# Gabrielcb/DaliID

Hardware: AMD Instinct MI355X
Metric: images/sec (train step) (higher is better)
Workload: dtype bf16; 1 GPU; configs[1]: ResNet-50 ReID bf16 256x128, PK batch 16x16=256 per GPU, center+proxy heads, Adam, EMA; global_batch=256, per_gpu_batch=256, parallelism=dp1

## Files before the change

daliid_amd/csrc/conv.hip:

```cpp
#include "gemm_tile.h"
#include "kernels.h"
#include <cstdlib>
#include <type_traits>
#include <vector>
#include <string>
#include <cstdio>

namespace dali {

__device__ __forceinline__ void decode_pixel(const GatherGeom& g, int p, int& n, int& ho, int& wo) {
    if (g.lhw >= 0 && g.lw >= 0) {
        n = p >> g.lhw;
        const int rem = p & ((1 << g.lhw) - 1);
        ho = rem >> g.lw;
        wo = rem & ((1 << g.lw) - 1);
    } else {
        const int hw = g.Hout * g.Wout;
        n = p / hw;
        const int rem = p - n * hw;
        ho = rem / g.Wout;
        wo = rem - ho * g.Wout;
    }
}

// ... 1049 lines not shown
        const uint16_t* sa = smem + (kt % NSTAGE) * A_ELEMS;
        const int kr = kt / 3, ks = kt - 3 * kr;
        const int tap_off = g.mode == 0 ? kr * HC + ks : (2 - kr) * HC + (2 - ks);
        uint32_t boff[FN];
#pragma unroll
        for (int j = 0; j < FN; ++j) {
            const int hp = hp_base[j] + tap_off;
            boff[j] = (uint32_t)(hp * 64 + (((lane >> 4) ^ ((hp >> 1) & 7)) << 3));
        }
#pragma unroll
        for (int h = 0; h < 2; ++h) {
            bf16x8_t fa[FM];
#pragma unroll
            for (int i = 0; i < FM; ++i) fa[i] = *reinterpret_cast<const bf16x8_t*>(sa + (i * 16) * 64 + (frag_off ^ (h << 5)));
#pragma unroll
            for (int j = 0; j < FN; ++j) {
                const bf16x8_t fb = *reinterpret_cast<const bf16x8_t*>(patch + (boff[j] ^ (uint32_t)(h << 5)));
#pragma unroll
                for (int i = 0; i < FM; ++i) acc[i][j] = __builtin_amdgcn_mfma_f32_16x16x32_bf16(fa[i], fb, acc[i][j], 0, 0, 0);
            }
        }
        asm volatile("s_waitcnt lgkmcnt(0)" ::: "memory");
        __builtin_amdgcn_s_barrier();
    }
    conv_epilogue_g<TM, TN, FM, FN, 4, NT, epi_mode(epi_fused(EPI), EPI)>(a, acc, 0, tn, smem, 0, wn);
}

}
#include "fused1x1.h"
namespace dali {

__device__ __forceinline__ int wg_swz(int row) { return (row & 3) | (((row >> 3) & 1) << 2); }

typedef short s16x4_t __attribute__((ext_vector_type(4)));

__device__ __forceinline__ int tr_frag_off(int chunk32, int lane, int half) {
    const int row = 8 * (lane >> 4) + ((lane & 15) >> 2) + 4 * half;
    return row * 128 + ((chunk32 ^ wg_swz(row)) << 4) + 4 * (lane & 3);
}
typedef short s16x8_t __attribute__((ext_vector_type(8)));
__device__ __forceinline__ bf16x8_t tr_frag(const uint16_t* tile, int chunk32, int lane) {
    typedef __attribute__((address_space(3))) s16x4_t* lds_ptr_t;
    const s16x4_t a = __builtin_amdgcn_ds_read_tr16_b64_v4i16((lds_ptr_t)(tile + tr_frag_off(chunk32, lane, 0)));
    const s16x4_t b = __builtin_amdgcn_ds_read_tr16_b64_v4i16((lds_ptr_t)(tile + tr_frag_off(chunk32, lane, 1)));
    return __builtin_bit_cast(bf16x8_t, s16x8_t{a[0], a[1], a[2], a[3], b[0], b[1], b[2], b[3]});
}

struct TrPair { s16x4_t lo, hi; };
__device__ __forceinline__ s16x4_t ds_read_tr_raw(const uint16_t* p) {
    typedef __attribute__((address_space(3))) const uint16_t* lds_cptr_t;
    const uint32_t addr = (uint32_t)(uintptr_t)(lds_cptr_t)p;
    s16x4_t v;
    asm volatile("ds_read_b64_tr_b16 %0, %1" : "=v"(v) : "v"(addr));
    return v;
}
__device__ __forceinline__ TrPair tr_frag_raw(const uint16_t* tile, int chunk32, int lane) {
    return TrPair{ds_read_tr_raw(tile + tr_frag_off(chunk32, lane, 0)), ds_read_tr_raw(tile + tr_frag_off(chunk32, lane, 1))};
}
__device__ __forceinline__ bf16x8_t tr_join(const TrPair& t) {
    return __builtin_bit_cast(bf16x8_t, s16x8_t{t.lo[0], t.lo[1], t.lo[2], t.lo[3], t.hi[0], t.hi[1], t.hi[2], t.hi[3]});
}
template <int N>
__device__ __forceinline__ void tr_settle(TrPair& a, TrPair& b, TrPair& c, TrPair& d) {
    static_assert(N == 0 || N == 8 || N == 10 || N == 16 || N == 18, "lgkmcnt immediates used by the callers");
    asm volatile("s_waitcnt lgkmcnt(%8)" : "+v"(a.lo), "+v"(a.hi), "+v"(b.lo), "+v"(b.hi), "+v"(c.lo), "+v"(c.hi), "+v"(d.lo), "+v"(d.hi) : "n"(N > 15 ? 15 : N));
}

__device__ __forceinline__ void tr_settle_all(TrPair& a) { asm volatile("s_waitcnt lgkmcnt(0)" : "+v"(a.lo), "+v"(a.hi)); }

template <int FM, int FN>
__device__ __forceinline__ void store_slab_tiles(float* slab, const f32x4_t (&acc)[FM][FN], int m_first, int n_first, int Cm, int Ntot, int lane) {
    const int mr = m_first + (lane >> 4) * 4, nc = n_first + (lane & 15);
    if (m_first + 16 * FM <= Cm && n_first + 16 * FN <= Ntot) {
        float* row = slab + (size_t)mr * Ntot + nc;
#pragma unroll
        for (int i = 0; i < FM; ++i)
#pragma unroll
            for (int rr = 0; rr < 4; ++rr) {
                float* p = row + (size_t)(i * 16 + rr) * Ntot;
#pragma unroll
                for (int j = 0; j < FN; ++j) p[j * 16] = acc[i][j][rr];
            }
        return;
    }
#pragma unroll
    for (int i = 0; i < FM; ++i)
#pragma unroll
        for (int j = 0; j < FN; ++j) {
            const int n = nc + j * 16;
#pragma unroll
            for (int rr = 0; rr < 4; ++rr) {
                const int m = mr + i * 16 + rr;
                if (m < Cm && n < Ntot) slab[(size_t)m * Ntot + n] = acc[i][j][rr];
// ... 1477 lines not shown
```

daliid_amd/csrc/gemm_tile.h:

```cpp
#pragma once
#include "common.h"

namespace dali {

__device__ __forceinline__ int lds_swz(int row) { return (0x1320 >> (((row >> 2) & 3) * 4)) & 3; }

template <int TM_, int TN_, int NA_, int NB_, int NPROD_>
struct GemmCfg {
    static constexpr int TM = TM_, TN = TN_, NA = NA_, NB = NB_, NPROD = NPROD_;
    static constexpr int BK = 32;
    static constexpr int FM = TM / 32, FN = TN / 32;
    static constexpr int A_ELEMS = TM * BK, B_ELEMS = TN * BK;
    static constexpr int STAGE_ELEMS = NA * A_ELEMS + NB * B_ELEMS;
    static constexpr int LDS_BYTES = 2 * STAGE_ELEMS * 2;
    static constexpr int ACH = TM * 4 / 256, BCH = TN * 4 / 256;
    static_assert(TM % 64 == 0 && TN % 64 == 0, "tile must be a multiple of 64");
    static_assert(NPROD == 1 || (NPROD == 3 && NA == 2 && NB == 2), "NPROD 3 needs hi/lo on both operands");
};

template <class Cfg, class LA, class LB>
__device__ __forceinline__ void gemm_mainloop(f32x4_t (&acc)[Cfg::FM][Cfg::FN], const LA& la, const LB& lb,
                                              int ktiles, uint16_t* smem) {
    constexpr int FM = Cfg::FM, FN = Cfg::FN, NA = Cfg::NA, NB = Cfg::NB;
    const int tid = threadIdx.x, lane = tid & 63, wave = tid >> 6;
// ... 64 lines not shown
                acc[i][j] = __builtin_amdgcn_mfma_f32_16x16x32_bf16(fa[0][i], fb[0], acc[i][j], 0, 0, 0);
                if constexpr (Cfg::NPROD == 3) {
                    acc[i][j] = __builtin_amdgcn_mfma_f32_16x16x32_bf16(fa[0][i], fb[1], acc[i][j], 0, 0, 0);
                    acc[i][j] = __builtin_amdgcn_mfma_f32_16x16x32_bf16(fa[1][i], fb[0], acc[i][j], 0, 0, 0);
                }
            }
        }
        if (more) sstore((kt + 1) & 1);
        __syncthreads();
    }
}

template <class Cfg>
__device__ __forceinline__ void acc_coords(int& m_base, int& n_base) {
    const int lane = threadIdx.x & 63, wave = threadIdx.x >> 6;
    m_base = (wave >> 1) * (Cfg::TM / 2) + (lane >> 4) * 4;
    n_base = (wave & 1) * (Cfg::TN / 2) + (lane & 15);
}

typedef __attribute__((address_space(3))) void* lds_void_ptr;
constexpr uint32_t DMA_OOB = 0x7ffffff0u;

template <int N>
__device__ __forceinline__ void vm_wait() {
    static_assert(N >= 0 && N <= 63, "vmcnt is a 6-bit field");
    asm volatile("s_waitcnt vmcnt(%0)" ::"n"(N) : "memory");
}
template <int N>
__device__ __forceinline__ void dma_wait() {
    static_assert(N == 0 || N == 2 || N == 3 || N == 4 || N == 5 || N == 6 || N == 8 || N == 9 || N == 10 || N == 12, "DMA piece counts of the rings in use");
    asm volatile("s_waitcnt vmcnt(%0) lgkmcnt(0)" ::"n"(N) : "memory");
}

__host__ __device__ __forceinline__ void xcd_super_shape(int tiles_m, int tiles_n, int& lg, int& ms) {
    const long long total = (long long)tiles_m * tiles_n;
    lg = total >= 1024 ? 6 : total >= 512 ? 5 : total >= 256 ? 4 : 3;
    ms = tiles_m >= 5 ? 3 : tiles_m >= 3 ? 2 : tiles_m == 2 ? 1 : 0;
    if (ms > lg) ms = lg;
}
__host__ __device__ __forceinline__ bool xcd_dense_map(int tiles_m, int ms) { return (tiles_m & ((1 << ms) - 1)) != 0; }
__device__ __forceinline__ bool xcd_tile_map(int b, int tiles_m, int tiles_n, int& tm, int& tn) {
    int lg, ms;
    xcd_super_shape(tiles_m, tiles_n, lg, ms);
    if (xcd_dense_map(tiles_m, ms)) {
        const int BM = tiles_m <= 16 ? tiles_m : 8;
        const int T = tiles_m * tiles_n, per = (T + 7) >> 3;
        const int xcd = b & 7, slot = b >> 3;
        const int t = xcd * per + slot;
        if (slot >= per || t >= T) return false;
        const int band_tiles = BM * tiles_n;
        const int band = t / band_tiles;
        const int r = t - band * band_tiles;
        const int left = tiles_m - band * BM;
        const int h = left < BM ? left : BM;
        tn = r / h;
        tm = band * BM + (r - tn * h);
        return true;
    }
    const int ns = lg - ms;
    const int xcd = b & 7, slot = b >> 3;
    const int ssn = (tiles_n + (1 << ns) - 1) >> ns;
    const int st = (slot >> lg) * 8 + xcd;
    const int w = slot & ((1 << lg) - 1);
    const int sm = st / ssn, sn = st - sm * ssn;
    tm = (sm << ms) + (w & ((1 << ms) - 1));
    tn = (sn << ns) + (w >> ms);
// ... 14 lines not shown
```

daliid_amd/csrc/kernels.h:

```cpp
#pragma once
#include "common.h"

namespace dali {

struct GatherGeom {
    int Hout, Wout;
    int Hin, Win;
    int Ck;
    int R, S, stride, pad;
    int mode;
    long long img_pitch;
    int row_pitch, pix_pitch;
    int lw, lhw;
    int sub, oph, opw, Hfull, Wfull;
    int r0, rstep, nr, s0, sstep, ns;
    int class_grid;
};

struct IGemmArgs {
    const uint16_t* W;
    const uint16_t* X;
    uint16_t* O;
    const uint16_t* Res;
    const uint8_t* res_mask;
// ... 60 lines not shown
int launch_bnlin_stats(hipStream_t st, const uint16_t* W, const uint16_t* Wt, const float* gram, const float* m2, int C, int w, double count, const float* gamma,
                       const float* beta, float* rm, float* rv, float momentum, float eps, float* ut, float* dot, float* scale, float* shift,
                       float* mean, float* invstd);
int launch_bnlin_ut(hipStream_t st, const uint16_t* W, const float* gram, int C, int w, float* ut);
int launch_bnlin_bwd(hipStream_t st, const uint16_t* W, const uint16_t* Wt, const float* ut, const float* m2, const float* s_dz, int C,
                     int w, double count, const float* scale, const float* mean, const float* invstd, float* dW, float* dgamma, float* dbeta,
                     uint16_t* wd1, uint16_t* wd2, float* bvec, float* qk, int ld1 = 0, int ld2 = 0);

constexpr int REDUCE_SMAX = 64;
inline size_t reduce_scratch_bytes(int C, int NV) { return (size_t)REDUCE_SMAX * C * NV * sizeof(double); }
int launch_bn_finalize(hipStream_t st, const float* partial, int tiles, int C, double count, const float* gamma, const float* beta,
                       float* rm, float* rv, float momentum, float eps, float* scale, float* shift, float* mean, float* invstd,
                       double* scratch);
struct BnEvalJob { const float *gamma, *beta, *rm, *rv; float *scale, *shift; int C; };
struct BnEvalJobs { static constexpr int MAX = 56; BnEvalJob job[MAX]; };
int launch_bn_eval_coeffs_batched(hipStream_t st, const BnEvalJob* jobs, int n, float eps);
int launch_fold_cat_weights(hipStream_t st, const float* w3, const float* wd, const float* s3, const float* sd, const float* h3, const float* hd, int C, int w,
                            int cin, int parts, uint16_t* wcat, float* shcat);
int launch_bn_act(hipStream_t st, const uint16_t* raw, const float* scale, const float* shift, const uint16_t* idn, const uint16_t* raw2,
                  const float* scale2, const float* shift2, int relu, size_t elems, int C, uint16_t* y, uint8_t* mask_out);
int bn_bwd_blocks(int P, int C, int* rows_per_block);
size_t bn_bwd_partial_floats(int P, int C, bool dual);
int launch_bn_bwd(hipStream_t st, const uint16_t* g, const uint16_t* ymask, const uint8_t* ybits, const BnBwdSide& a, const BnBwdSide* b, int relu, int P, int C,
                  float* partial, float* coef_a, float* coef_b, float* dgamma_a, float* dbeta_a, float* dgamma_b, float* dbeta_b,
                  uint16_t* draw_a, uint16_t* draw_b, uint16_t* dz_out, double* scratch);
int launch_stem_pack_image(hipStream_t st, const float* img, int N, int H, int W, uint16_t* out);
int launch_stem_pack_weight(hipStream_t st, const float* w, int Cout, uint16_t* out);
bool stem_fused_supported(int N, int H, int W, int C);
bool stem_train_supported(int N, int H, int W, int C);
int stem_train_tiles(int N, int H);
int launch_stem_conv_stats(hipStream_t st, const uint16_t* ximg, const uint16_t* w_packed, int N, int H, int W, uint16_t* raw, float* stats);
int launch_stem_conv_bn_pool(hipStream_t st, const uint16_t* ximg, const uint16_t* w_packed, const float* scale, const float* shift, int N, int H, int W,
                             uint16_t* out);
int launch_stem_unpack_wgrad(hipStream_t st, const float* padded, int Cout, float* dw);
int launch_maxpool_bn_fwd(hipStream_t st, const uint16_t* raw, const float* scale, const float* shift, int N, int H, int W, int C,
                          uint16_t* out, uint8_t* arg);
int maxpool_bn_bwd_blocks(int N, int H, int W, int C, int* quads_per_block);
int launch_maxpool_bn_bwd(hipStream_t st, const uint16_t* dp, const uint8_t* arg, const uint16_t* raw, const float* mean, const float* invstd,
                          const float* scale, int N, int H, int W, int C, float* partial, float* coef, float* dgamma, float* dbeta,
                          uint16_t* draw, double* scratch);
int launch_head_pool_fwd(hipStream_t st, const uint16_t* x, int N, int HW, int C, int mode, float* f, int16_t* arg);
int launch_head_pool_bwd(hipStream_t st, const float* df, const int16_t* arg, int N, int HW, int C, int mode, uint16_t* dx, const uint8_t* ybits = nullptr);
int launch_bn1d_fwd(hipStream_t st, const float* x, int N, int C, const float* gamma, const float* beta, float* rm, float* rv, int training,
                    float momentum, float eps, float* y, float* mean, float* invstd);
int launch_bn1d_bwd(hipStream_t st, const float* x, const float* dy, int N, int C, const float* gamma, const float* mean, const float* invstd,
                    float* dx, float* dgamma, float* dbeta);
int launch_cast_bf16(hipStream_t st, const float* x, size_t n, uint16_t* y);
int launch_weight_transpose(hipStream_t st, const uint16_t* w, int Co, int T, int Ci, uint16_t* wt);


int launch_patchify(hipStream_t st, const float* img, int B, int H, int W, int ps, int stride, uint16_t* out);
int launch_assemble_tokens(hipStream_t st, const uint16_t* pe, const float* cls, const float* pos, int B, int T, int C, uint16_t* x);
int launch_assemble_tokens_bwd(hipStream_t st, const uint16_t* dx, int B, int T, int C, float* dpos, float* dcls, uint16_t* dpe);
int launch_layernorm_fwd(hipStream_t st, const uint16_t* x, const float* gamma, const float* beta, int rows, int C, float eps,
                         uint16_t* y, float* mean, float* rstd, float* y32);
size_t layernorm_bwd_partial_floats(int rows, int C);
int launch_layernorm_bwd(hipStream_t st, const uint16_t* g, const uint16_t* x, const float* gamma, const float* mean, const float* rstd,
                         const uint16_t* add, int rows, int C, uint16_t* dx, float* dgamma, float* dbeta, float* partial, double* scratch,
                         const float* g32 = nullptr);
size_t colsum_partial_floats(int rows, int C);
int launch_colsum(hipStream_t st, const uint16_t* y, int rows, int C, float* out, float* partial, double* scratch);
int launch_rowscale_add(hipStream_t st, const uint16_t* branch, const float* scale, int samples, int rows_per_sample, int C, const uint16_t* res,
                        uint16_t* out);
int launch_expand_rowscale(hipStream_t st, const float* scale, int n_vec, int B, int T, float* out);
int launch_attention_fwd(hipStream_t st, const uint16_t* qkv, int B, int T, int H, float scale, uint16_t* out, float* lse);
int launch_attention_fwd_short(hipStream_t st, const uint16_t* qkv, int B, int T, int H, float scale, uint16_t* out, float* lse);
// ... 19 lines not shown
```

daliid_amd/csrc/resnet_plan.hip:

```cpp
#include "kernels.h"
#include <cstdio>
#include <cstring>
#include <new>
#include <string>
#include <vector>

using namespace dali;

namespace {

struct TensorInfo { std::string name; int64_t offset, numel; int shape[4]; int ndim; };

struct Conv {
    int cin, cout, r, s, stride, pad, hin, win, hout, wout;
    int64_t w_off;
    uint16_t* w_bf16;
    uint16_t* wt_bf16;
};
struct Bn {
    int C;
    int64_t g_off, b_off;
    int64_t rm_off, rv_off;
    float *scale, *shift, *mean, *invstd, *coef;
};
// ... 83 lines not shown
}

template <class T>
void reserve(dali_resnet* net, Arena& a, T*& ptr, size_t bytes) {
    net->fixups.emplace_back(reinterpret_cast<void**>(&ptr), a.take(bytes));
}
void reserve_bn(dali_resnet* net, Arena& a, Bn& b) {
    reserve(net, a, b.scale, b.C * 4); reserve(net, a, b.shift, b.C * 4);
    reserve(net, a, b.mean, b.C * 4); reserve(net, a, b.invstd, b.C * 4);
    reserve(net, a, b.coef, b.C * 12);
}

int conv_halo_w(const Conv& c) {
    const bool pow2 = (c.wout & (c.wout - 1)) == 0 && ((c.hout * c.wout) & (c.hout * c.wout - 1)) == 0;
    return (c.r == 3 && c.s == 3 && c.stride == 1 && c.pad == 1 && pow2 && c.hout * c.wout >= 128) ? c.wout : 0;
}
GatherGeom conv_geom(const Conv& c, int mode) {
    GatherGeom g{};
    if (mode == 0) {
        g.Hout = c.hout; g.Wout = c.wout; g.Hin = c.hin; g.Win = c.win; g.Ck = c.cin;
    } else {
        g.Hout = c.hin; g.Wout = c.win; g.Hin = c.hout; g.Win = c.wout; g.Ck = c.cout;
    }
    g.R = c.r; g.S = c.s; g.stride = c.stride; g.pad = c.pad; g.mode = mode;
    g.pix_pitch = g.Ck; g.row_pitch = g.Win * g.Ck; g.img_pitch = (long long)g.Hin * g.Win * g.Ck;
    g.lw = g.lhw = -1;
    return g;
}
Conv square_conv(const Conv& c3) {
    Conv q = c3;
    q.cin = c3.cin; q.cout = c3.cin; q.w_off = 0; q.w_bf16 = nullptr; q.wt_bf16 = nullptr;
    return q;
}
GatherGeom stem_geom(const dali_resnet* net) {
    GatherGeom g{};
    g.Hout = net->stem_h; g.Wout = net->stem_w;
    g.Hin = net->H + 6; g.Win = net->W + 8;
    g.Ck = 32; g.R = 7; g.S = 1; g.stride = 2; g.pad = 0; g.mode = 0;
    g.pix_pitch = 4; g.row_pitch = (net->W + 8) * 4; g.img_pitch = (long long)(net->H + 6) * (net->W + 8) * 4;
    g.lw = g.lhw = -1;
    return g;
}

}

extern "C" int dali_resnet_create(dali_ctx* ctx, const dali_resnet_cfg* cfg, dali_resnet** out) {
    DALI_REQUIRE(ctx && cfg && out, "dali_resnet_create: null argument");
    DALI_REQUIRE(cfg->batch > 0 && cfg->height >= 32 && cfg->width >= 32 && cfg->height % 32 == 0 && cfg->width % 16 == 0,
                 "dali_resnet_create: bad input shape %dx%dx%d (height %% 32, width %% 16)", cfg->batch, cfg->height, cfg->width);
    DALI_REQUIRE(cfg->width_base >= 32 && cfg->width_base % 32 == 0 && cfg->width_base <= 64,
                 "dali_resnet_create: width_base must be 32 or 64 (got %d)", cfg->width_base);
    for (int i = 0; i < 4; ++i) DALI_REQUIRE(cfg->layers[i] >= 1, "dali_resnet_create: layers[%d] < 1", i);
    dali_resnet* net = new (std::nothrow) dali_resnet();
    if (!net) { set_error("dali_resnet_create: out of host memory"); return DALI_ERR_NOMEM; }
    net->ctx = ctx; net->cfg = *cfg; net->N = cfg->batch; net->H = cfg->height; net->W = cfg->width;
    const int wb = cfg->width_base;
    add_conv(net, net->stem, "conv1", 3, wb, 7, 2, 3, net->H, net->W);
    add_bn(net, net->stem_bn, "bn1", wb);
    net->stem_h = net->stem.hout; net->stem_w = net->stem.wout;
    net->pool_h = (net->stem_h + 2 - 3) / 2 + 1; net->pool_w = (net->stem_w + 2 - 3) / 2 + 1;
    int h = net->pool_h, w = net->pool_w, inpl = wb;
    const int strides[4] = {1, 2, 2, 1};
    for (int li = 0; li < 4; ++li) {
        const int planes = wb << li;
        net->stage_first[li] = (int)net->blocks.size();
        for (int bi = 0; bi < cfg->layers[li]; ++bi) {
            Block b{};
            const int st = bi == 0 ? strides[li] : 1;
            const std::string pre = "layer" + std::to_string(li + 1) + "." + std::to_string(bi);
            b.hin = h; b.win = w; b.cin = inpl; b.width = planes; b.cout = planes * 4;
            add_conv(net, b.c1, pre + ".conv1", inpl, planes, 1, 1, 0, h, w);
            add_bn(net, b.b1, pre + ".bn1", planes);
            add_conv(net, b.c2, pre + ".conv2", planes, planes, 3, st, 1, h, w);
            add_bn(net, b.b2, pre + ".bn2", planes);
            add_conv(net, b.c3, pre + ".conv3", planes, planes * 4, 1, 1, 0, b.c2.hout, b.c2.wout);
// ... 3 lines not shown
                add_conv(net, b.cd, pre + ".downsample.0", inpl, planes * 4, 1, st, 0, h, w);
                add_bn(net, b.bd, pre + ".downsample.1", planes * 4);
            }
            b.hout = b.c2.hout; b.wout = b.c2.wout;
            b.lin_ds = b.has_ds && st == 1 && inpl % 32 == 0 && inpl <= 128 && net->blocks.empty();
            h = b.hout; w = b.wout; inpl = planes * 4;
            net->blocks.push_back(b);
        }
        net->stage_last[li] = (int)net->blocks.size() - 1;
    }
    net->feat_dim = inpl;
    net->head_hw = h * w;
    DALI_REQUIRE(net->head_hw < 32768, "dali_resnet_create: final map too large");
    add_bn(net, net->neck, "last_bn", net->feat_dim);

    Arena a;
    const size_t N = net->N;
    reserve(net, a, net->wbf16_flat, (size_t)net->param_elems * 2);
    reserve(net, a, net->w_stem, (size_t)wb * 224 * 2);
    reserve(net, a, net->ximg, N * (net->H + 6) * (net->W + 8) * 4 * 2);
    const size_t raw0_bytes = N * net->stem_h * net->stem_w * wb * 2;
    reserve(net, a, net->raw0, raw0_bytes);
    reserve(net, a, net->pool0, N * net->pool_h * net->pool_w * wb * 2);
    reserve(net, a, net->pool_arg, N * net->pool_h * net->pool_w * wb);
    reserve_bn(net, a, net->stem_bn);
    size_t max_act = raw0_bytes, max_stat = (size_t)igemm_conv_stat_tiles(wb, (int)N * net->stem_h * net->stem_w, 224) * wb * 2 * 4;
    int stem_qpb;
    size_t max_bwd_partial = (size_t)maxpool_bn_bwd_blocks((int)N, net->stem_h, net->stem_w, wb, &stem_qpb) * wb * 2 * 4;
    size_t max_slab = 0, max_cs = 256;
    {
        int sp, pps; size_t wsb;
        wgrad_plan(wb, 224, (int)N * net->stem_h * net->stem_w, 512, &sp, &pps, &wsb, 7);
        max_slab = wsb;
    }
    for (auto& b : net->blocks) {
        const size_t pin = N * b.hin * b.win, pout = N * b.hout * b.wout;
        reserve(net, a, b.raw1, pin * b.width * 2);
        reserve(net, a, b.a1, pin * b.width * 2);
        reserve(net, a, b.raw2, pout * b.width * 2);
        reserve(net, a, b.a2, pout * b.width * 2);
        reserve(net, a, b.gram, (size_t)b.width * b.width * 4); reserve(net, a, b.m2, (size_t)b.width * 4);
        reserve(net, a, b.sdz, (size_t)b.cout * 4); reserve(net, a, b.bvec, (size_t)b.width * 4); reserve(net, a, b.qk, (size_t)b.cout * 8);
        reserve(net, a, b.wd1, (size_t)b.width * (b.cout + b.width) * 2);
        reserve(net, a, b.ut, (size_t)b.width * b.cout * 4); reserve(net, a, b.dot, (size_t)(b.width / 32) * b.cout * 12);
        max_cs = std::max(max_cs, std::max(colsum_partial_floats((int)pout, b.cout), colsum_partial_floats((int)pout, b.width)) * 4);
        int sp, pps; size_t wsb;
        wgrad_plan(b.width, b.width, (int)pout, 512, &sp, &pps, &wsb, 1, 0);
        max_slab = std::max(max_slab, wsb);
        max_cs = std::max(max_cs, (size_t)wgrad_colsum_rows(b.width, b.width, 1, (int)pout, sp) * b.width * 4);
        wgrad_plan(b.cout, b.width, (int)pout, 512, &sp, &pps, &wsb, 1, 0);
        max_cs = std::max(max_cs, (size_t)wgrad_colsum_rows(b.cout, b.width, 1, (int)pout, sp) * b.cout * 4);
        reserve(net, a, b.y, pout * b.cout * 2);
        reserve(net, a, b.ybits, pout * b.cout / 8);
        if (b.has_ds) reserve(net, a, b.rawd, pout * b.cout * 2);
        if (b.lin_ds) {
            reserve(net, a, b.gram_d, (size_t)b.cin * b.cin * 4); reserve(net, a, b.m2_d, (size_t)b.cin * 4);
            reserve(net, a, b.ut_d, (size_t)b.cin * b.cout * 4); reserve(net, a, b.bvec_d, (size_t)b.cin * 4); reserve(net, a, b.qk_d, (size_t)b.cout * 8);
            reserve(net, a, b.wdd, (size_t)b.cin * (b.cout + b.cin) * 2);
            int sp, pps; size_t wsb;
            wgrad_plan(b.cin, b.cin, (int)pin, 512, &sp, &pps, &wsb, 1, 0);
            max_slab = std::max(max_slab, wsb);
            max_cs = std::max(max_cs, std::max(colsum_partial_floats((int)pin, b.cin), (size_t)wgrad_colsum_rows(b.cin, b.cin, 1, (int)pin, sp) * b.cin) * 4);
        }
        b.cat_eval = b.has_ds && b.cd.stride == 1 && conv_cat_act_supported(b.cout, b.width, b.cin, (int)pout, 2);
        if (b.cat_eval) { reserve(net, a, b.wcat, (size_t)b.cout * 2 * (b.width + b.cin) * 2); reserve(net, a, b.shcat, (size_t)b.cout * 4); }
        reserve_bn(net, a, b.b1); reserve_bn(net, a, b.b2); reserve_bn(net, a, b.b3);
// ... 320 lines not shown
    BnBwdSide s1{b.raw1, b.b1.mean, b.b1.invstd, b.b1.scale, b.b1.shift};
    if ((rc = launch_bn_bwd(st, d_a1, nullptr, nullptr, s1, nullptr, 1, Pin, b.width, net->bwd_partial, b.b1.coef, nullptr, net->G + b.b1.g_off,
                            net->G + b.b1.b_off, nullptr, nullptr, d_a1, nullptr, nullptr, net->red_scratch))) return rc;
    b.dbg_d_raw1 = d_a1;
    if ((rc = conv_wgrad(net, st, b.c1, b.x, nullptr, d_a1))) return rc;
    uint16_t* dx = d_a2;
    if (b.lin_ds) {
        if ((rc = conv_dgrad(net, st, b.c1, d_a1, nullptr, dx, prev_bits))) return rc;
        Conv cat = b.cd;
        cat.cout = b.cout + b.cin;
        IGemmArgs ga{};
        ga.W = b.wdd; ga.X = dz; ga.X2 = b.x; ga.Ck1 = b.cout; ga.O = dx; ga.Res = dx; ga.bias = b.bvec_d;
        ga.Cm = b.cin; ga.P = Pin;
        ga.g = conv_geom(cat, 1);
        if ((rc = launch_igemm_conv(st, ga))) return rc;
    } else if (b.has_ds) {
        if ((rc = conv_wgrad(net, st, b.cd, b.x, nullptr, d_rawd))) return rc;
        if ((rc = conv_dgrad(net, st, b.c1, d_a1, nullptr, dx, prev_bits))) return rc;
        if ((rc = conv_dgrad(net, st, b.cd, d_rawd, dx, dx, prev_bits))) return rc;
    } else {
        if ((rc = conv_dgrad(net, st, b.c1, d_a1, dz, dx, prev_bits))) return rc;
    }
    net->cur_dy = dx;
    net->cur_dy_bytes = (int64_t)Pin * b.cin * 2;
    return DALI_OK;
}

static int stem_backward(dali_resnet* net, hipStream_t st) {
    int rc;
    uint16_t* d_raw0 = next_gbuf(net, net->cur_dy);
    if ((rc = launch_maxpool_bn_bwd(st, net->cur_dy, net->pool_arg, net->raw0, net->stem_bn.mean, net->stem_bn.invstd, net->stem_bn.scale,
                                    net->N, net->stem_h, net->stem_w, net->stem.cout, net->bwd_partial, net->stem_bn.coef,
                                    net->G + net->stem_bn.g_off, net->G + net->stem_bn.b_off, d_raw0, net->red_scratch))) return rc;
    WGradArgs a{};
    a.dY = d_raw0; a.X = net->ximg; a.partial = net->wgrad_slab; a.in_scale = nullptr; a.in_shift = nullptr; a.in_relu = 0;
    a.Cm = net->stem.cout; a.P = net->N * net->stem_h * net->stem_w; a.Ntot = 224;
    a.g = stem_geom(net);
    size_t wsb;
    wgrad_plan(a.Cm, a.Ntot, a.P, 512, &a.splits, &a.pix_per_split, &wsb, 7);
    if ((rc = launch_igemm_wgrad(st, a, net->stem_dw_pad, 0))) return rc;
    return launch_stem_unpack_wgrad(st, net->stem_dw_pad, net->stem.cout, net->G + net->stem.w_off);
}

extern "C" int dali_resnet_backward(dali_resnet* net, void* stream, const float* d_emb, int stage_begin, int stage_end) {
    DALI_REQUIRE(net && net->P && net->G, "dali_resnet_backward: net not bound (grads required)");
    DALI_REQUIRE(net->fwd_training, "dali_resnet_backward: the last forward was not in training mode");
    DALI_REQUIRE(stage_begin >= 0 && stage_end <= 3 && stage_begin <= stage_end, "dali_resnet_backward: bad stage range %d..%d", stage_begin, stage_end);
    hipStream_t st = (hipStream_t)stream;
    int rc;
    for (int stage = stage_begin; stage <= stage_end; ++stage) {
        const int li = 3 - stage;
        if (stage == 0) {
            DALI_REQUIRE(d_emb != nullptr, "dali_resnet_backward: d_emb is null");
            if ((rc = launch_bn1d_bwd(st, net->feat, d_emb, net->N, net->feat_dim, net->P + net->neck.g_off, net->neck_mean, net->neck_invstd,
                                      net->dfeat, net->G + net->neck.g_off, net->G + net->neck.b_off))) return rc;
            net->cur_dy = net->gbuf[0];
            if ((rc = launch_head_pool_bwd(st, net->dfeat, net->head_arg, net->N, net->head_hw, net->feat_dim, net->feature_mode, net->cur_dy,
                                           net->blocks.back().ybits))) return rc;
            net->cur_dy_bytes = (int64_t)net->N * net->head_hw * net->feat_dim * 2;
        }
        for (int bi = net->stage_last[li]; bi >= net->stage_first[li]; --bi)
            if ((rc = block_backward(net, st, net->blocks[bi], bi > 0 ? net->blocks[bi - 1].ybits : nullptr))) return rc;
        if (stage == 3 && (rc = stem_backward(net, st))) return rc;
    }
    return DALI_OK;
}
// ... 61 lines not shown
```

daliid_amd/csrc/stem.hip:

```cpp
#include "common.h"
#include "kernels.h"
#include "gemm_tile.h"

namespace dali {
namespace {

typedef short s16x2_t __attribute__((ext_vector_type(2)));
__device__ __forceinline__ uint32_t order_key2(uint32_t x) {
    const s16x2_t v = __builtin_bit_cast(s16x2_t, x);
    const s16x2_t m = {(short)0x7FFF, (short)0x7FFF};
    return __builtin_bit_cast(uint32_t, (s16x2_t)(v ^ ((v >> 15) & m)));
}
__device__ __forceinline__ uint32_t max_key2(uint32_t a, uint32_t b) {
    return __builtin_bit_cast(uint32_t, __builtin_elementwise_max(__builtin_bit_cast(s16x2_t, a), __builtin_bit_cast(s16x2_t, b)));
}
__device__ __forceinline__ uint4 max_key8(uint4 a, uint4 b) {
    return make_uint4(max_key2(a.x, b.x), max_key2(a.y, b.y), max_key2(a.z, b.z), max_key2(a.w, b.w));
}

struct StemArgs {
    const uint16_t* ximg;
    const uint16_t* w;
    const float* scale; const float* shift;
    uint16_t* out;
// ... 229 lines not shown
                for (int i = 0; i < 4; ++i) acc[i] = __builtin_amdgcn_mfma_f32_16x16x32_bf16(A[i][r], B[r], acc[i], 0, 0, 0);
            const int px = cr * a.Wc + wc0 + n16;
#pragma unroll
            for (int h = 0; h < 2; ++h) {
                uint32_t k[4];
#pragma unroll
                for (int p = 0; p < 4; ++p) {
                    const int e = 8 * h + 2 * p;
                    const float v0 = acc[e >> 2][e & 3], v1 = acc[(e + 1) >> 2][(e + 1) & 3];
                    s1[e] += v0; s2[e] += v0 * v0; s1[e + 1] += v1; s2[e + 1] += v1 * v1;
                    k[p] = pack_bf16x2(v0, v1);
                }
                *reinterpret_cast<uint4*>(rtile + px * 128 + (((2 * q + h) ^ (px & 7)) << 4)) = make_uint4(k[0], k[1], k[2], k[3]);
            }
        }
#pragma unroll
        for (int e = 0; e < 16; ++e) { s1[e] = st_row16_sum(s1[e]); s2[e] = st_row16_sum(s2[e]); }
        if (n16 == 0) {
#pragma unroll
            for (int e = 0; e < 16; ++e) { wstat[wave * 128 + (16 * q + e) * 2] = s1[e]; wstat[wave * 128 + (16 * q + e) * 2 + 1] = s2[e]; }
        }
        asm volatile("s_waitcnt lgkmcnt(0)" ::: "memory");
        __builtin_amdgcn_s_barrier();
        if (more) deposit(sf_smem + (buf ^ 1) * patch_pitch, st);
        if (t + 2 * (int)gridDim.x < a.tiles) request(t + 2 * gridDim.x, st);
        asm volatile("" ::: "memory");
        uint16_t* dst = a.raw + (size_t)t * (ST_CONV_ROWS * a.Wc * 64);
        for (int c = tid; c < ST_CONV_ROWS * a.Wc * 8; c += SF_THREADS) {
            const int px = c >> 3, cc = c & 7;
            *reinterpret_cast<uint4*>(dst + (size_t)c * 8) = *reinterpret_cast<const uint4*>(rtile + px * 128 + ((cc ^ (px & 7)) << 4));
        }
        if (tid < 128) a.stats[(size_t)t * 128 + tid] = ((wstat[tid] + wstat[128 + tid]) + wstat[256 + tid]) + wstat[384 + tid];
    }
}

int stem_cu_count() {
    static int n_cus = 0;
    if (!n_cus) {
        int dev = 0, v = 0;
        if (hipGetDevice(&dev) != hipSuccess || hipDeviceGetAttribute(&v, hipDeviceAttributeMultiprocessorCount, dev) != hipSuccess) return -1;
        n_cus = v > 0 ? v : 1;
    }
    return n_cus;
}

}

bool stem_train_supported(int N, int H, int W, int C) {
    if (C != 64 || W != 128 || H % 8 != 0) return false;
    if ((long long)N * (H + 6) * (W + 8) * 8 >= 0x7ff00000ll) return false;
    return DALI_ENV_INT("DALI_TRAIN_STEM", 1) != 0;
}
int stem_train_tiles(int N, int H) { return N * (H / 2 / 4); }
int launch_stem_conv_stats(hipStream_t st, const uint16_t* ximg, const uint16_t* w, int N, int H, int W, uint16_t* raw, float* stats) {
    if (!stem_train_supported(N, H, W, 64)) { set_error("stem_conv_stats: unsupported shape %d x %d x %d", N, H, W); return DALI_ERR_INVALID; }
    StemTrainArgs a{};
    a.ximg = ximg; a.w = w; a.raw = raw; a.stats = stats;
    a.N = N; a.Hp = H + 6; a.Wp = W + 8; a.Hc = H / 2; a.Wc = W / 2; a.tiles = stem_train_tiles(N, H);
    const int lds = 2 * SF_THREADS * SF_NST * 16 + ST_CONV_ROWS * a.Wc * 128 + 4 * 128 * 4;
    DALI_ONCE_PER_DEVICE(DALI_HIP(hipFuncSetAttribute(reinterpret_cast<const void*>(&stem_conv_stats_kernel), hipFuncAttributeMaxDynamicSharedMemorySize, 80 * 1024)));
    const int n_cus = stem_cu_count();
    if (n_cus <= 0) { set_error("stem_conv_stats: device query failed"); return DALI_ERR_HIP; }
    const int grid = a.tiles < 2 * n_cus ? a.tiles : 2 * n_cus;
    char what[160];
    snprintf(what, sizeof what, "fwd,Cm=64,K=224,P=%d,taps=7,stride=2,sub=0,fused=0,stats=1,res=0,mask=0,lin=0", N * a.Hc * a.Wc);
    const int slot = gemm_profile_begin(st, 0, 2.0 * 64 * 224 * (double)N * a.Hc * a.Wc, what);
    hipLaunchKernelGGL(stem_conv_stats_kernel, dim3(grid), dim3(SF_THREADS), lds, st, a);
    gemm_profile_end(st, slot);
    DALI_LAUNCH_CHECK();
    return DALI_OK;
}

bool stem_fused_supported(int N, int H, int W, int C) {
    if (C != 64 || H % 32 != 0 || !(W == 32 || W == 64 || W == 128)) return false;
    const int Wp = W + 8, Hp = H + 6;
    if (SF_PATCH_ROWS * Wp * 8 / 16 > SF_THREADS * SF_NST) return false;
    if ((long long)N * Hp * Wp * 8 >= 0x7ff00000ll) return false;
    return DALI_ENV_INT("DALI_EVAL_STEM", 1) != 0;
}

int launch_stem_conv_bn_pool(hipStream_t st, const uint16_t* ximg, const uint16_t* w, const float* scale, const float* shift, int N, int H, int W,
                             uint16_t* out) {
    if (!stem_fused_supported(N, H, W, 64)) { set_error("stem_conv_bn_pool: unsupported shape %d x %d x %d", N, H, W); return DALI_ERR_INVALID; }
    StemArgs a{};
    a.ximg = ximg; a.w = w; a.scale = scale; a.shift = shift; a.out = out;
    a.N = N; a.Hp = H + 6; a.Wp = W + 8; a.Wc = W / 2; a.Ho = H / 4; a.Wo = W / 4;
    a.tiles = N * (a.Ho / 2);
    a.lwo = W == 32 ? 3 : (W == 64 ? 4 : 5);
    const int lds = 2 * SF_THREADS * SF_NST * 16 + SF_CONV_ROWS * a.Wc * 128 + 512;
    DALI_ONCE_PER_DEVICE(DALI_HIP(hipFuncSetAttribute(reinterpret_cast<const void*>(&stem_conv_bn_pool_kernel), hipFuncAttributeMaxDynamicSharedMemorySize, 80 * 1024)));
    const int n_cus = stem_cu_count();
    if (n_cus <= 0) { set_error("stem_conv_bn_pool: device query failed"); return DALI_ERR_HIP; }
    const int grid = a.tiles < 2 * n_cus ? a.tiles : 2 * n_cus;
    hipLaunchKernelGGL(stem_conv_bn_pool_kernel, dim3(grid), dim3(SF_THREADS), lds, st, a);
    DALI_LAUNCH_CHECK();
    return DALI_OK;
}

}

extern "C" int dali_stem_fused_supported(int n, int h, int w) { return dali::stem_fused_supported(n, h, w, 64) ? 1 : 0; }

extern "C" int dali_stem_conv_bn_maxpool(dali_ctx* ctx, void* stream, const float* images, int n, int h, int w, const float* weight, const float* scale,
                                         const float* shift, uint16_t* y) {
    using namespace dali;
    DALI_REQUIRE(ctx && images && weight && scale && shift && y, "dali_stem_conv_bn_maxpool: null argument");
    DALI_REQUIRE(n > 0 && stem_fused_supported(n, h, w, 64), "dali_stem_conv_bn_maxpool: unsupported shape %d x %d x %d (dali_stem_fused_supported)", n, h, w);
    const size_t img_bytes = align_up((size_t)n * (h + 6) * (w + 8) * 8, 256);
    unsigned char* ws = static_cast<unsigned char*>(workspace(ctx, img_bytes + 64 * 224 * 2));
    if (!ws) return DALI_ERR_NOMEM;
    hipStream_t st = (hipStream_t)stream;
    uint16_t* ximg = reinterpret_cast<uint16_t*>(ws);
    uint16_t* wp = reinterpret_cast<uint16_t*>(ws + img_bytes);
    int rc;
    if ((rc = launch_stem_pack_image(st, images, n, h, w, ximg))) return rc;
    if ((rc = launch_stem_pack_weight(st, weight, 64, wp))) return rc;
    return launch_stem_conv_bn_pool(st, ximg, wp, scale, shift, n, h, w, y);
}
```

include/daliid_debug.h:

```cpp
#ifndef DALIID_DEBUG_H
#define DALIID_DEBUG_H

#ifdef __cplusplus
extern "C" {
#endif

int dali_debug_reload_env(void);

int dali_debug_set_conv_stamps(void* dev_ptr);

int dali_debug_wgrad_splits(int Cm, int Ntot, int P, int taps, int halo_w);

int dali_debug_splitk_reduce(void* stream, const float* partial, float* out, long long elems, int splits, int accumulate);

struct dali_resnet;
int dali_debug_resnet_backward_block(struct dali_resnet* net, void* stream, const float* d_emb, int block);

#ifdef __cplusplus
}
#endif
#endif
```

Measured before the change: 17750 images/s.

## Add dedicated stem weight-gradient kernel using LDS patch staging and transposed reads

Adds a specialized stem conv weight-gradient kernel for W=128. It stages the input image patch and the dY tile in LDS, reads them with ds_read_b64_tr_b16 at immediate offsets, and software-pipelines the fragment loads across 8 k-steps feeding MFMAs. Each block writes a per-block slab, and a split-K reduce then sums the slabs. The kernel replaces the generic gathered implicit-GEMM wgrad in the backward pass to cut gather overhead, at the cost of an extra reduction over roughly 2*CUs slabs and extra slab memory.

```diff
diff --git a/daliid_amd/csrc/conv.hip b/daliid_amd/csrc/conv.hip
--- a/daliid_amd/csrc/conv.hip
+++ b/daliid_amd/csrc/conv.hip
@@ -1105,13 +1105,10 @@
 
 __device__ __forceinline__ int wg_swz(int row) { return (row & 3) | (((row >> 3) & 1) << 2); }
 
-typedef short s16x4_t __attribute__((ext_vector_type(4)));
-
 __device__ __forceinline__ int tr_frag_off(int chunk32, int lane, int half) {
     const int row = 8 * (lane >> 4) + ((lane & 15) >> 2) + 4 * half;
     return row * 128 + ((chunk32 ^ wg_swz(row)) << 4) + 4 * (lane & 3);
 }
-typedef short s16x8_t __attribute__((ext_vector_type(8)));
 __device__ __forceinline__ bf16x8_t tr_frag(const uint16_t* tile, int chunk32, int lane) {
     typedef __attribute__((address_space(3))) s16x4_t* lds_ptr_t;
     const s16x4_t a = __builtin_amdgcn_ds_read_tr16_b64_v4i16((lds_ptr_t)(tile + tr_frag_off(chunk32, lane, 0)));
@@ -1119,19 +1116,8 @@
     return __builtin_bit_cast(bf16x8_t, s16x8_t{a[0], a[1], a[2], a[3], b[0], b[1], b[2], b[3]});
 }
 
-struct TrPair { s16x4_t lo, hi; };
-__device__ __forceinline__ s16x4_t ds_read_tr_raw(const uint16_t* p) {
-    typedef __attribute__((address_space(3))) const uint16_t* lds_cptr_t;
-    const uint32_t addr = (uint32_t)(uintptr_t)(lds_cptr_t)p;
-    s16x4_t v;
-    asm volatile("ds_read_b64_tr_b16 %0, %1" : "=v"(v) : "v"(addr));
-    return v;
-}
 __device__ __forceinline__ TrPair tr_frag_raw(const uint16_t* tile, int chunk32, int lane) {
     return TrPair{ds_read_tr_raw(tile + tr_frag_off(chunk32, lane, 0)), ds_read_tr_raw(tile + tr_frag_off(chunk32, lane, 1))};
-}
-__device__ __forceinline__ bf16x8_t tr_join(const TrPair& t) {
-    return __builtin_bit_cast(bf16x8_t, s16x8_t{t.lo[0], t.lo[1], t.lo[2], t.lo[3], t.hi[0], t.hi[1], t.hi[2], t.hi[3]});
 }
 template <int N>
 __device__ __forceinline__ void tr_settle(TrPair& a, TrPair& b, TrPair& c, TrPair& d) {
diff --git a/daliid_amd/csrc/gemm_tile.h b/daliid_amd/csrc/gemm_tile.h
--- a/daliid_amd/csrc/gemm_tile.h
+++ b/daliid_amd/csrc/gemm_tile.h
@@ -120,6 +120,30 @@
     asm volatile("s_waitcnt vmcnt(%0) lgkmcnt(0)" ::"n"(N) : "memory");
 }
 
+typedef short s16x4_t __attribute__((ext_vector_type(4)));
+typedef short s16x8_t __attribute__((ext_vector_type(8)));
+struct TrPair { s16x4_t lo, hi; };
+__device__ __forceinline__ uint32_t lds_addr_of(const void* p) {
+    typedef __attribute__((address_space(3))) const unsigned char* lds_cptr_t;
+    return (uint32_t)(uintptr_t)(lds_cptr_t)p;
+}
+__device__ __forceinline__ s16x4_t ds_read_tr_raw(const uint16_t* p) {
+    const uint32_t addr = lds_addr_of(p);
+    s16x4_t v;
+    asm volatile("ds_read_b64_tr_b16 %0, %1" : "=v"(v) : "v"(addr));
+    return v;
+}
+template <int OFF>
+__device__ __forceinline__ s16x4_t ds_read_tr_raw_at(uint32_t addr) {
+    static_assert(OFF >= 0 && OFF < 65536 && OFF % 8 == 0, "16-bit offset field, 8-byte aligned reads");
+    s16x4_t v;
+    asm volatile("ds_read_b64_tr_b16 %0, %1 offset:%2" : "=v"(v) : "v"(addr), "n"(OFF));
+    return v;
+}
+__device__ __forceinline__ bf16x8_t tr_join(const TrPair& t) {
+    return __builtin_bit_cast(bf16x8_t, s16x8_t{t.lo[0], t.lo[1], t.lo[2], t.lo[3], t.hi[0], t.hi[1], t.hi[2], t.hi[3]});
+}
+
 __host__ __device__ __forceinline__ void xcd_super_shape(int tiles_m, int tiles_n, int& lg, int& ms) {
     const long long total = (long long)tiles_m * tiles_n;
     lg = total >= 1024 ? 6 : total >= 512 ? 5 : total >= 256 ? 4 : 3;
diff --git a/daliid_amd/csrc/kernels.h b/daliid_amd/csrc/kernels.h
--- a/daliid_amd/csrc/kernels.h
+++ b/daliid_amd/csrc/kernels.h
@@ -116,6 +116,11 @@
 int launch_stem_conv_stats(hipStream_t st, const uint16_t* ximg, const uint16_t* w_packed, int N, int H, int W, uint16_t* raw, float* stats);
 int launch_stem_conv_bn_pool(hipStream_t st, const uint16_t* ximg, const uint16_t* w_packed, const float* scale, const float* shift, int N, int H, int W,
                              uint16_t* out);
+bool stem_wgrad_shape_ok(int N, int H, int W, int C);
+size_t stem_wgrad_slab_bytes(int N, int H);
+int launch_stem_wgrad(hipStream_t st, const uint16_t* ximg, const uint16_t* dy, int N, int H, int W, float* slab, float* dw_pad);
+GatherGeom stem_gather_geom(int H, int W);
+int launch_stem_wgrad_gathered(hipStream_t st, const uint16_t* ximg, const uint16_t* dy, int N, int H, int W, float* slab, float* dw_pad);
 int launch_stem_unpack_wgrad(hipStream_t st, const float* padded, int Cout, float* dw);
 int launch_maxpool_bn_fwd(hipStream_t st, const uint16_t* raw, const float* scale, const float* shift, int N, int H, int W, int C,
                           uint16_t* out, uint8_t* arg);
diff --git a/daliid_amd/csrc/resnet_plan.hip b/daliid_amd/csrc/resnet_plan.hip
--- a/daliid_amd/csrc/resnet_plan.hip
+++ b/daliid_amd/csrc/resnet_plan.hip
@@ -139,15 +139,7 @@
     q.cin = c3.cin; q.cout = c3.cin; q.w_off = 0; q.w_bf16 = nullptr; q.wt_bf16 = nullptr;
     return q;
 }
-GatherGeom stem_geom(const dali_resnet* net) {
-    GatherGeom g{};
-    g.Hout = net->stem_h; g.Wout = net->stem_w;
-    g.Hin = net->H + 6; g.Win = net->W + 8;
-    g.Ck = 32; g.R = 7; g.S = 1; g.stride = 2; g.pad = 0; g.mode = 0;
-    g.pix_pitch = 4; g.row_pitch = (net->W + 8) * 4; g.img_pitch = (long long)(net->H + 6) * (net->W + 8) * 4;
-    g.lw = g.lhw = -1;
-    return g;
-}
+GatherGeom stem_geom(const dali_resnet* net) { return stem_gather_geom(net->H, net->W); }
 
 }
 
@@ -217,6 +209,7 @@
         int sp, pps; size_t wsb;
         wgrad_plan(wb, 224, (int)N * net->stem_h * net->stem_w, 512, &sp, &pps, &wsb, 7);
         max_slab = wsb;
+        if (stem_wgrad_shape_ok((int)N, net->H, net->W, wb)) max_slab = std::max(max_slab, stem_wgrad_slab_bytes((int)N, net->H));
     }
     for (auto& b : net->blocks) {
         const size_t pin = N * b.hin * b.win, pout = N * b.hout * b.wout;
@@ -603,6 +596,10 @@
     if ((rc = launch_maxpool_bn_bwd(st, net->cur_dy, net->pool_arg, net->raw0, net->stem_bn.mean, net->stem_bn.invstd, net->stem_bn.scale,
                                     net->N, net->stem_h, net->stem_w, net->stem.cout, net->bwd_partial, net->stem_bn.coef,
                                     net->G + net->stem_bn.g_off, net->G + net->stem_bn.b_off, d_raw0, net->red_scratch))) return rc;
+    if (stem_train_supported(net->N, net->H, net->W, net->stem.cout)) {
+        if ((rc = launch_stem_wgrad(st, net->ximg, d_raw0, net->N, net->H, net->W, net->wgrad_slab, net->stem_dw_pad))) return rc;
+        return launch_stem_unpack_wgrad(st, net->stem_dw_pad, net->stem.cout, net->G + net->stem.w_off);
+    }
     WGradArgs a{};
     a.dY = d_raw0; a.X = net->ximg; a.partial = net->wgrad_slab; a.in_scale = nullptr; a.in_shift = nullptr; a.in_relu = 0;
     a.Cm = net->stem.cout; a.P = net->N * net->stem_h * net->stem_w; a.Ntot = 224;
diff --git a/daliid_amd/csrc/stem.hip b/daliid_amd/csrc/stem.hip
--- a/daliid_amd/csrc/stem.hip
+++ b/daliid_amd/csrc/stem.hip
@@ -285,6 +285,123 @@
         }
         if (tid < 128) a.stats[(size_t)t * 128 + tid] = ((wstat[tid] + wstat[128 + tid]) + wstat[256 + tid]) + wstat[384 + tid];
     }
+}
+
+struct StemWgradArgs {
+    const uint16_t* ximg;
+    const uint16_t* dy;
+    float* slab;
+    int N, Hp, Hc, tiles;
+};
+constexpr int SW_ROW_BYTES = (128 + 8) * 8;
+constexpr int SW_PATCH_BYTES = SF_THREADS * SF_NST * 16;
+constexpr int SW_DY_BYTES = ST_CONV_ROWS * 64 * 128, SW_DY_NST = SW_DY_BYTES / 16 / SF_THREADS;
+static_assert(ST_PATCH_ROWS * SW_ROW_BYTES <= SW_PATCH_BYTES, "the patch fits its staging slots");
+__device__ __forceinline__ int sw_swz(int px) { return ((px >> 1) & 1) | (((px >> 3) & 1) << 1); }
+
+struct SwFrags { TrPair a[2], b[7]; };
+template <int KS>
+__device__ __forceinline__ void sw_issue(SwFrags& f, const uint32_t (&a_addr)[2], uint32_t b_addr) {
+#pragma unroll
+    for (int m = 0; m < 2; ++m) {
+        f.a[m].lo = ds_read_tr_raw_at<KS * 4096>(a_addr[m]);
+        f.a[m].hi = ds_read_tr_raw_at<KS * 4096 + 512>(a_addr[m]);
+    }
+    constexpr int B0 = 2 * (KS >> 1) * SW_ROW_BYTES + (KS & 1) * 512;
+    f.b[0].lo = ds_read_tr_raw_at<B0>(b_addr);                        f.b[0].hi = ds_read_tr_raw_at<B0 + 64>(b_addr);
+    f.b[1].lo = ds_read_tr_raw_at<B0 + 1 * SW_ROW_BYTES>(b_addr);     f.b[1].hi = ds_read_tr_raw_at<B0 + 1 * SW_ROW_BYTES + 64>(b_addr);
+    f.b[2].lo = ds_read_tr_raw_at<B0 + 2 * SW_ROW_BYTES>(b_addr);     f.b[2].hi = ds_read_tr_raw_at<B0 + 2 * SW_ROW_BYTES + 64>(b_addr);
+    f.b[3].lo = ds_read_tr_raw_at<B0 + 3 * SW_ROW_BYTES>(b_addr);     f.b[3].hi = ds_read_tr_raw_at<B0 + 3 * SW_ROW_BYTES + 64>(b_addr);
+    f.b[4].lo = ds_read_tr_raw_at<B0 + 4 * SW_ROW_BYTES>(b_addr);     f.b[4].hi = ds_read_tr_raw_at<B0 + 4 * SW_ROW_BYTES + 64>(b_addr);
+    f.b[5].lo = ds_read_tr_raw_at<B0 + 5 * SW_ROW_BYTES>(b_addr);     f.b[5].hi = ds_read_tr_raw_at<B0 + 5 * SW_ROW_BYTES + 64>(b_addr);
+    f.b[6].lo = ds_read_tr_raw_at<B0 + 6 * SW_ROW_BYTES>(b_addr);     f.b[6].hi = ds_read_tr_raw_at<B0 + 6 * SW_ROW_BYTES + 64>(b_addr);
+}
+__device__ __forceinline__ void sw_settle(SwFrags& f) {
+    asm volatile("s_waitcnt lgkmcnt(0)"
+                 : "+v"(f.a[0].lo), "+v"(f.a[0].hi), "+v"(f.a[1].lo), "+v"(f.a[1].hi), "+v"(f.b[0].lo), "+v"(f.b[0].hi), "+v"(f.b[1].lo), "+v"(f.b[1].hi),
+                   "+v"(f.b[2].lo), "+v"(f.b[2].hi), "+v"(f.b[3].lo), "+v"(f.b[3].hi), "+v"(f.b[4].lo), "+v"(f.b[4].hi), "+v"(f.b[5].lo), "+v"(f.b[5].hi),
+                   "+v"(f.b[6].lo), "+v"(f.b[6].hi));
+}
+__device__ __forceinline__ void sw_mma(f32x4_t (&acc)[2][7], const SwFrags& f) {
+    const bf16x8_t a0 = tr_join(f.a[0]), a1 = tr_join(f.a[1]);
+#pragma unroll
+    for (int r = 0; r < 7; ++r) {
+        const bf16x8_t b = tr_join(f.b[r]);
+        acc[0][r] = __builtin_amdgcn_mfma_f32_16x16x32_bf16(a0, b, acc[0][r], 0, 0, 0);
+        acc[1][r] = __builtin_amdgcn_mfma_f32_16x16x32_bf16(a1, b, acc[1][r], 0, 0, 0);
+    }
+}
+template <int KS>
+__device__ __forceinline__ void sw_tile(f32x4_t (&acc)[2][7], SwFrags& cur, SwFrags& nxt, const uint32_t (&a_addr)[2], uint32_t b_addr) {
+    sw_settle(cur);
+    if constexpr (KS + 1 < 8) sw_issue<KS + 1>(nxt, a_addr, b_addr);
+    sw_mma(acc, cur);
+    if constexpr (KS + 1 < 8) sw_tile<KS + 1>(acc, nxt, cur, a_addr, b_addr);
+}
+
+__global__ __launch_bounds__(SF_THREADS, 2) void stem_wgrad_kernel(StemWgradArgs a) {
+    extern __shared__ __attribute__((aligned(16))) unsigned char sf_smem[];
+    const int tid = threadIdx.x, lane = tid & 63;
+    const int wave = __builtin_amdgcn_readfirstlane(tid >> 6);
+    const int mh = wave & 1, jh = wave >> 1;
+    const int g = lane >> 4, q = (lane & 15) >> 2, p4 = lane & 3;
+    unsigned char* patch = sf_smem;
+    unsigned char* ytile = sf_smem + SW_PATCH_BYTES;
+    constexpr int nchunks = ST_PATCH_ROWS * SW_ROW_BYTES >> 4;
+    const __amdgpu_buffer_rsrc_t rs_x = __builtin_amdgcn_make_buffer_rsrc(const_cast<uint16_t*>(a.ximg), 0, a.N * a.Hp * SW_ROW_BYTES, 0x00020000);
+    const __amdgpu_buffer_rsrc_t rs_y = __builtin_amdgcn_make_buffer_rsrc(const_cast<uint16_t*>(a.dy), 0, a.tiles * SW_DY_BYTES, 0x00020000);
+    const int tiles_per_img = a.Hc >> 2;
+    uint4 sx[SF_NST], sy[SW_DY_NST];
+    auto request = [&](int t) {
+        const int n = t / tiles_per_img, r4 = t - n * tiles_per_img;
+        const int base = (n * a.Hp + 8 * r4) * SW_ROW_BYTES;
+#pragma unroll
+        for (int s = 0; s < SF_NST; ++s) {
+            const int c = tid + SF_THREADS * s;
+            const uint32_t off = (uint32_t)(base + c * 16) | (c < nchunks ? 0u : DMA_OOB);
+            sx[s] = __builtin_bit_cast(uint4, __builtin_amdgcn_raw_buffer_load_b128(rs_x, off, 0, 0));
+        }
+#pragma unroll
+        for (int s = 0; s < SW_DY_NST; ++s)
+            sy[s] = __builtin_bit_cast(uint4, __builtin_amdgcn_raw_buffer_load_b128(rs_y, (uint32_t)(t * SW_DY_BYTES + (tid + SF_THREADS * s) * 16), 0, 0));
+    };
+    const int ydst = (tid >> 3) * 128 + ((((tid & 7) >> 1) ^ sw_swz(tid >> 3)) << 5) + ((tid & 1) << 4);
+    auto deposit = [&]() {
+#pragma unroll
+        for (int s = 0; s < SF_NST; ++s) *reinterpret_cast<uint4*>(patch + (tid + SF_THREADS * s) * 16) = sx[s];
+#pragma unroll
+        for (int s = 0; s < SW_DY_NST; ++s) *reinterpret_cast<uint4*>(ytile + ydst + s * 4096) = sy[s];
+    };
+    uint32_t a_addr[2];
+#pragma unroll
+    for (int m = 0; m < 2; ++m) a_addr[m] = lds_addr_of(ytile) + (8 * g + q) * 128 + (((2 * mh + m) ^ sw_swz(8 * g + q)) << 5) + 8 * p4;
+    const uint32_t b_addr = lds_addr_of(patch) + (8 * g + q) * 16 + jh * 32 + 8 * p4;
+
+    f32x4_t acc[2][7];
+#pragma unroll
+    for (int m = 0; m < 2; ++m)
+#pragma unroll
+        for (int r = 0; r < 7; ++r) acc[m][r] = f32x4_t{0.f, 0.f, 0.f, 0.f};
+    int t = blockIdx.x;
+    request(t);
+    for (; t < a.tiles; t += gridDim.x) {
+        deposit();
+        if (t + (int)gridDim.x < a.tiles) request(t + gridDim.x);
+        asm volatile("s_waitcnt lgkmcnt(0)" ::: "memory");
+        __builtin_amdgcn_s_barrier();
+        SwFrags f0, f1;
+        sw_issue<0>(f0, a_addr, b_addr);
+        sw_tile<0>(acc, f0, f1, a_addr, b_addr);
+        asm volatile("s_waitcnt lgkmcnt(0)" ::: "memory");
+        __builtin_amdgcn_s_barrier();
+    }
+    float* slab = a.slab + (size_t)blockIdx.x * (64 * 224);
+#pragma unroll
+    for (int m = 0; m < 2; ++m)
+#pragma unroll
+        for (int r = 0; r < 7; ++r)
+#pragma unroll
+            for (int i = 0; i < 4; ++i) slab[(16 * (2 * mh + m) + 4 * g + i) * 224 + 32 * r + 16 * jh + (lane & 15)] = acc[m][r][i];
 }
 
 int stem_cu_count() {
@@ -324,6 +441,36 @@
     return DALI_OK;
 }
 
+bool stem_wgrad_shape_ok(int N, int H, int W, int C) {
+    if (N <= 0 || C != 64 || W != 128 || H <= 0 || H % 8 != 0) return false;
+    return (long long)N * (H + 6) * (W + 8) * 8 < 0x7ff00000ll && (long long)N * (H / 2) * (W / 2) * 128 < 0x7ff00000ll;
+}
+static int stem_wgrad_grid(int N, int H) {
+    const int n_cus = stem_cu_count(), tiles = stem_train_tiles(N, H);
+    if (n_cus <= 0) return -1;
+    return tiles < 2 * n_cus ? tiles : 2 * n_cus;
+}
+size_t stem_wgrad_slab_bytes(int N, int H) {
+    const int grid = stem_wgrad_grid(N, H);
+    return grid > 0 ? (size_t)grid * 64 * 224 * sizeof(float) : 0;
+}
+int launch_stem_wgrad(hipStream_t st, const uint16_t* ximg, const uint16_t* dy, int N, int H, int W, float* slab, float* dw_pad) {
+    if (!stem_wgrad_shape_ok(N, H, W, 64)) { set_error("stem_wgrad: unsupported shape %d x %d x %d", N, H, W); return DALI_ERR_INVALID; }
+    StemWgradArgs a{};
+    a.ximg = ximg; a.dy = dy; a.slab = slab;
+    a.N = N; a.Hp = H + 6; a.Hc = H / 2; a.tiles = stem_train_tiles(N, H);
+    const int grid = stem_wgrad_grid(N, H);
+    if (grid <= 0) { set_error("stem_wgrad: device query failed"); return DALI_ERR_HIP; }
+    const int P = N * a.Hc * (W / 2);
+    char what[160];
+    snprintf(what, sizeof what, "wgrad,Cm=64,K=224,P=%d,taps=7,stride=2,sub=0,fused=0,stats=0,res=0,mask=0,lin=0", P);
+    const int slot = gemm_profile_begin(st, 1, 2.0 * 64 * 224 * (double)P, what);
+    hipLaunchKernelGGL(stem_wgrad_kernel, dim3(grid), dim3(SF_THREADS), SW_PATCH_BYTES + SW_DY_BYTES, st, a);
+    gemm_profile_end(st, slot);
+    DALI_LAUNCH_CHECK();
+    return launch_splitk_reduce(st, slab, dw_pad, (size_t)64 * 224, grid, 0);
+}
+
 bool stem_fused_supported(int N, int H, int W, int C) {
     if (C != 64 || H % 32 != 0 || !(W == 32 || W == 64 || W == 128)) return false;
     const int Wp = W + 8, Hp = H + 6;
@@ -370,3 +517,51 @@
     if ((rc = launch_stem_pack_weight(st, weight, 64, wp))) return rc;
     return launch_stem_conv_bn_pool(st, ximg, wp, scale, shift, n, h, w, y);
 }
+
+namespace dali {
+GatherGeom stem_gather_geom(int H, int W) {
+    GatherGeom g{};
+    g.Hout = (H + 6 - 7) / 2 + 1; g.Wout = (W + 6 - 7) / 2 + 1;
+    g.Hin = H + 6; g.Win = W + 8;
+    g.Ck = 32; g.R = 7; g.S = 1; g.stride = 2; g.pad = 0; g.mode = 0;
+    g.pix_pitch = 4; g.row_pitch = (W + 8) * 4; g.img_pitch = (long long)(H + 6) * (W + 8) * 4;
+    g.lw = g.lhw = -1;
+    return g;
+}
+int launch_stem_wgrad_gathered(hipStream_t st, const uint16_t* ximg, const uint16_t* dy, int N, int H, int W, float* slab, float* dw_pad) {
+    WGradArgs a{};
+    a.dY = dy; a.X = ximg; a.partial = slab;
+    a.g = stem_gather_geom(H, W);
+    a.Cm = 64; a.P = N * a.g.Hout * a.g.Wout; a.Ntot = 224;
+    size_t wsb;
+    wgrad_plan(a.Cm, a.Ntot, a.P, 512, &a.splits, &a.pix_per_split, &wsb, 7);
+    return launch_igemm_wgrad(st, a, dw_pad, 0);
+}
+}
+
+extern "C" int dali_debug_stem_wgrad(dali_ctx* ctx, void* stream, const float* images, const uint16_t* d_raw0, int n, int h, int w, int path, float* dw_out) {
+    using namespace dali;
+    DALI_REQUIRE(ctx && images && d_raw0 && dw_out, "dali_debug_stem_wgrad: null argument");
+    DALI_REQUIRE(n > 0 && h > 0 && w > 0 && h % 2 == 0 && w % 2 == 0 && (path == 0 || path == 1), "dali_debug_stem_wgrad: bad argument");
+    DALI_REQUIRE(path == 1 || stem_wgrad_shape_ok(n, h, w, 64), "dali_debug_stem_wgrad: the patch kernel takes W = 128, H %% 8 == 0 (got %d x %d x %d)", n, h, w);
+    size_t slab_bytes = 0;
+    if (path == 0) {
+        slab_bytes = stem_wgrad_slab_bytes(n, h);
+        DALI_REQUIRE(slab_bytes > 0, "dali_debug_stem_wgrad: device query failed");
+    } else {
+        int sp, pps;
+        wgrad_plan(64, 224, n * (h / 2) * (w / 2), 512, &sp, &pps, &slab_bytes, 7);
+    }
+    const size_t img_bytes = align_up((size_t)n * (h + 6) * (w + 8) * 8, 256);
+    slab_bytes = align_up(slab_bytes, 256);
+    unsigned char* ws = static_cast<unsigned char*>(workspace(ctx, img_bytes + slab_bytes + 64 * 224 * 4));
+    if (!ws) return DALI_ERR_NOMEM;
+    hipStream_t st = (hipStream_t)stream;
+    uint16_t* ximg = reinterpret_cast<uint16_t*>(ws);
+    float* slab = reinterpret_cast<float*>(ws + img_bytes);
+    float* dw_pad = reinterpret_cast<float*>(ws + img_bytes + slab_bytes);
+    int rc;
+    if ((rc = launch_stem_pack_image(st, images, n, h, w, ximg))) return rc;
+    if ((rc = path == 0 ? launch_stem_wgrad(st, ximg, d_raw0, n, h, w, slab, dw_pad) : launch_stem_wgrad_gathered(st, ximg, d_raw0, n, h, w, slab, dw_pad))) return rc;
+    return launch_stem_unpack_wgrad(st, dw_pad, 64, dw_out);
+}
diff --git a/include/daliid_debug.h b/include/daliid_debug.h
--- a/include/daliid_debug.h
+++ b/include/daliid_debug.h
@@ -1,5 +1,7 @@
 #ifndef DALIID_DEBUG_H
 #define DALIID_DEBUG_H
+
+#include <stdint.h>
 
 #ifdef __cplusplus
 extern "C" {
@@ -16,6 +18,9 @@
 struct dali_resnet;
 int dali_debug_resnet_backward_block(struct dali_resnet* net, void* stream, const float* d_emb, int block);
 
+struct dali_ctx;
+int dali_debug_stem_wgrad(struct dali_ctx* ctx, void* stream, const float* images, const uint16_t* d_raw0, int n, int h, int w, int path, float* dw_out);
+
 #ifdef __cplusplus
 }
 #endif
```

Measured after the change: 17820 images/s (median of 6 runs). Within noise of the previous version (+0.4%).
